# tier4/icp_rust

Hardware: AMD Instinct MI355X
Metric: ICP iterations/sec on 1M-pt 3D pair (higher is better)
Workload: dtype f64

## Files before the change

icp_rust_amd/_lib.py:

```python
import ctypes as C
import os
import subprocess

_HERE = os.path.dirname(os.path.abspath(__file__))
_CSRC = os.path.join(_HERE, "csrc")
LIB_PATH = os.environ.get("ICP_MI355X_LIB") or os.path.join(_HERE, "lib", "libicp_mi355x.so")

OK, NONE, EMPTY_DST, NAN_INPUT, BAD_ARGUMENT, NO_DEVICE, HIP_ERROR, OUT_OF_MEMORY, RETRY_REPLICATED, RETRY_SHARDED = range(10)
NN_AUTO, NN_BRUTE, NN_GRID = 0, 1, 2


class Pose(C.Structure):

    _fields_ = [(n, C.c_double) for n in ("r00", "r10", "r01", "r11", "tx", "ty")]

    def as_tuple(self):
        return (self.r00, self.r10, self.r01, self.r11, self.tx, self.ty)


class BatchItem(C.Structure):

    _fields_ = [("src_first", C.c_uint64), ("n", C.c_uint64), ("dst_first", C.c_uint64), ("m", C.c_uint64),
                ("init", Pose)]

# ... 86 lines not shown
    "icp_estimate_transform_device": (C.c_int, [_vp, _vp, _vp, _sz, _pp, _vp]),
    "icp_nn_search_device": (C.c_int, [_vp, _vp, _sz, _vp]),
    "icp_weighted_gn_step_device": (C.c_int, [_vp, _vp, _vp, _sz, _pp, C.c_int, _dp, _dp]),
    "icp_shard_geometry": (C.c_int, [_sz, C.c_int, C.c_int, C.POINTER(C.c_int), C.POINTER(C.c_int),
                                     C.POINTER(C.c_int), C.POINTER(_sz)]),
    "icp_shard_histogram_words": (_sz, []),
    "icp_shard_candidates_bytes": (_sz, []),
    "icp_shard_partials_bytes": (_sz, [C.c_int]),
    "icp_shard_exchange_bytes": (_sz, [C.c_int]),
    "icp_shard_take_device": (C.c_int, [_vp, _vp, _vp, _sz, C.c_int, C.c_int, _sz]),
    "icp_shard_put_device": (C.c_int, [_vp, _vp, _vp, _sz, C.c_int, C.c_int, _sz]),
    "icp_shard_eval_hist_device": (C.c_int, [_vp, _vp, _vp, _sz, C.c_int, C.c_int, _pp, C.c_int, C.c_int,
                                             C.POINTER(_vp)]),
    "icp_shard_eval_compact_device": (C.c_int, [_vp, _vp]),
    "icp_shard_eval_finish_device": (C.c_int, [_vp, _vp, _dp, _dp]),
    "icp_create_multi": (C.c_int, [C.POINTER(_vp), C.c_int, _vp, _sz, C.POINTER(C.c_int), C.c_int]),
    "icp_multi_estimate": (C.c_int, [_vp, _vp, _sz, _pp, _sz, _pp, _vp, _vp]),
    "icp_multi_counters": (C.c_int, [_vp, C.POINTER(C.c_uint64)]),
    "icp_multi_loop_counters": (C.c_int, [_vp, C.POINTER(C.c_uint64)]),
    "icp_multi_pipe_iterations": (C.c_int, [_vp, C.POINTER(C.c_uint64)]),
    "icp_pipe_counters": (C.c_int, [_vp, C.POINTER(C.c_uint64)]),
    "icp_debug_sort_cells": (C.c_int, [_vp, _sz, C.c_uint, _vp, _vp]),
    "icp_set_fixed_point_exit": (C.c_int, [_vp, C.c_int]),
    "icp_shard_pipe_run_device": (C.c_int, [_vp, _vp, _sz, _sz, C.c_int, C.c_int, _pp, C.POINTER(_sz), _sz, _vp, _vp,
                                            C.POINTER(C.c_int)]),
    "icp_loop_inbox_bytes": (_sz, []),
    "icp_loop_inbox": (C.c_int, [_vp, C.c_int, C.POINTER(C.c_void_p)]),
    "icp_loop_inbox_ipc_handle": (C.c_int, [_vp, C.c_char_p]),
    "icp_loop_ipc_open": (C.c_int, [C.c_int, C.c_char_p, C.POINTER(C.c_void_p)]),
    "icp_loop_ipc_close": (C.c_int, [_vp]),
    "icp_loop_inbox_shm_name": (C.c_int, [_vp, C.c_char_p]),
    "icp_loop_inbox_shm_unlink": (C.c_int, [_vp]),
    "icp_loop_shm_open": (C.c_int, [C.c_int, C.c_char_p, C.POINTER(C.c_void_p)]),
    "icp_loop_shm_close": (C.c_int, [_vp]),
    "icp_loop_transport_probe": (C.c_int, [_vp, C.c_int, C.POINTER(C.c_int)]),
    "icp_reset_window_predictions": (C.c_int, [_vp]),
    "icp_shard_loop_connect": (C.c_int, [_vp, C.c_int, C.c_int, C.POINTER(C.c_void_p)]),
    "icp_shard_loop_launch_device": (C.c_int, [_vp, _vp, _vp, _sz, C.c_uint, C.c_uint, C.c_int, C.c_uint32, _pp, C.c_double,
                                               C.c_int, C.c_int]),
    "icp_shard_loop_wait": (C.c_int, [_vp, _pp, C.POINTER(C.c_double), _u32p, C.POINTER(C.c_int), C.POINTER(C.c_int), _u32p]),
    "icp_destroy_multi": (None, [_vp]),
    "icp_synchronize": (C.c_int, [_vp]),
    "icp_profile_enable": (C.c_int, [_vp, C.c_int]),
    "icp_profile_read": (C.c_int, [_vp, _dp, C.POINTER(C.c_uint64)]),
    "icp_reduce_geometry": (None, [_sz, C.POINTER(C.c_int), C.POINTER(C.c_int)]),
    "icp_nn_cert_counters": (C.c_int, [_vp, C.POINTER(C.c_uint64)]),
# ... 97 lines not shown
```

icp_rust_amd/csrc/api.hip:

```cpp
#include <dlfcn.h>
#include <fcntl.h>
#include <sys/mman.h>
#include <unistd.h>

#include <cfloat>
#include <chrono>
#include <cstdio>
#include <cstring>
#include <atomic>
#include <map>
#include <mutex>
#include <new>

#include "api_internal.hpp"

using namespace icp;
using namespace icp::api;

namespace icp {
namespace api {
int map_hip(hipError_t e) {
  switch (e) {
    case hipSuccess: return ICP_OK;
    case hipErrorOutOfMemory: return ICP_OUT_OF_MEMORY;
// ... 1255 lines not shown
    if (rc != ICP_OK) return rc;
  }
  out[0] = h->ws.win_tried;
  out[1] = h->ws.win_missed;
  out[2] = h->ws.short_evals;
  out[3] = h->ws.radix_evals;
  out[4] = h->ws.spec_hits;
  out[5] = h->ws.spec_misses;
  return ICP_OK;
}

extern "C" int icp_gn_filed_counters(icp_handle *h, uint64_t out[2]) {
  if (!out) return ICP_BAD_ARGUMENT;
  std::lock_guard<std::mutex> lk(g_scratch_mu);
  if (!h) {
    const int rc = scratch_handle(&h);
    if (rc != ICP_OK) return rc;
  }
  out[0] = h->ws.bkt_evals;
  out[1] = h->ws.bkt_off;
  return ICP_OK;
}

extern "C" int icp_run_ahead_counters(icp_handle *h, uint64_t out[2]) {
  if (!h || !out) return ICP_BAD_ARGUMENT;
  out[0] = h->ws.ahead_hits;
  out[1] = h->ws.ahead_misses;
  return ICP_OK;
}

extern "C" int icp_gn_loop_timeouts(icp_handle *h, uint64_t *out) {
  if (!h || !out) return ICP_BAD_ARGUMENT;
  *out = h->ws.loop_timeouts;
  return ICP_OK;
}

extern "C" int icp_fixed_point_skips(icp_handle *h, uint64_t *out) {
  if (!h || !out) return ICP_BAD_ARGUMENT;
  *out = h->ws.fixed_point_skips;
  return ICP_OK;
}

extern "C" int icp_gn_loop_counters(icp_handle *h, uint64_t out[3]) {
  if (!out) return ICP_BAD_ARGUMENT;
  std::lock_guard<std::mutex> lk(g_scratch_mu);
  if (!h) {
// ... 98 lines not shown
```

icp_rust_amd/csrc/common.hpp:

```cpp
#pragma once
#include <hip/hip_runtime.h>

#include <cstddef>
#include <cstdint>
#include <cstdlib>
#include <utility>
#include <vector>

#include "pose.hpp"

namespace icp {


struct Range {
  explicit Range(const char *name);
  ~Range();
  Range(const Range &) = delete;
  Range &operator=(const Range &) = delete;
};

constexpr int kReduceThreads = 512;
constexpr int kReduceMaxBlocks = 256;
constexpr int kTreeMaxBlocks = 2048;
constexpr int kShardMaxWorld = 16;
// ... 152 lines not shown
  uint32_t *d_idx_slot = nullptr;
  double *d_sa = nullptr, *d_sb = nullptr;
  uint32_t *h_whist = nullptr;
  void *h_tiny = nullptr;
  unsigned long long tiny_calls = 0, tiny_evals = 0, tiny_sorted = 0;
  double *d_rlist = nullptr;
  unsigned *d_rlist_len = nullptr;
  size_t cap_part = 0;
  double *d_part_d = nullptr;
  uint32_t *d_part_i = nullptr;
  bool win_valid = false;
  bool win_wide = false;
  double win_med[2] = {0., 0.}, win_sigma[2] = {0., 0.};
  struct WinPred {
    bool valid = false, wide = false;
    double med[2] = {0., 0.}, sigma[2] = {0., 0.};
  };
  WinPred win_kind[5];
  WinPred hint_kind[5];
  uint32_t hint_last_inner = 0xffffffffu;
  static bool kind_has_slot(int kind) { return kind == 0 || kind == 1 || kind == 3 || kind == 4; }
  unsigned long long win_tried = 0, win_missed = 0, short_evals = 0, radix_evals = 0;
  unsigned long long bkt_evals = 0, bkt_misses = 0;
  unsigned long long fixed_point_skips = 0;
  unsigned bkt_off = 0;
  void *d_loop_ctl = nullptr, *h_loop_res = nullptr;
  uint32_t *d_loop_hist = nullptr;
  double *d_loop_part = nullptr;
  unsigned loop_seq = 0;
  bool loop_off = false;
  unsigned long long loop_launches = 0, loop_evals = 0, loop_handbacks = 0, loop_timeouts = 0;
  void *d_loop_inbox = nullptr;
  int loop_inbox_kind = 0;
  void *loop_inbox_host = nullptr;
  char loop_shm_name[64] = {0};
  unsigned loop_probe_gen = 0;
  unsigned loop_off_calls = 0;
  void *loop_peers[kShardMaxWorld] = {};
  int loop_rank = -1, loop_world = 0;
  void *loop_plan = nullptr;
  unsigned pipe_gen = 0;
  unsigned long long pipe_iters = 0, pipe_handbacks = 0, pipe_gave_up = 0;
  unsigned pipe_off = 0;
};

struct GridParams {
// ... 66 lines not shown
  bool have_prev = false;
  PrevMatch *d_prev = nullptr;
  double *d_sorted = nullptr;
  bool have_certs = false, have_pose = false, have_pose_before = false;
  double decay_r = 0., decay_t = 0.;
  Pose last_pose;
  uint32_t *d_cert_lists = nullptr;
  unsigned *d_cert_ctr = nullptr, *last_cert_ctr = nullptr;
  unsigned cert_seq = 0;
  unsigned long long cert_searches = 0;
};

hipError_t stable_sort_cells(const uint32_t *keys_in, uint32_t *perm_out, unsigned n, unsigned bits, void *&tmp, size_t &cap_tmp,
                             hipStream_t s);

}

struct icp_handle {
  int dim = 0;
  size_t m = 0;
  int device = 0;
  int nn_mode = ICP_NN_AUTO;
  bool single_launch = true;
  bool fixed_point_exit = true;
  bool owns_dst = false;
  const double *d_dst = nullptr;
  double *d_dst_own = nullptr;
  size_t cap_dst_own = 0, cap_soa = 0, cap_f32 = 0;
  double *d_dst_soa = nullptr;
  float *d_dst_f32 = nullptr;
  size_t m_pad = 0;
  bool brute_valid = false;
  bool screen_valid = false;
  hipStream_t own_stream = nullptr;
  hipStream_t stream = nullptr;
  icp::Workspace ws;
  icp::Grid grid;
  icp::QuerySort qsort;
  struct ShardEval {
    icp::WinParams P;
    int kind = 2, rank = 0, world = 1, b0 = 0, b1 = 0, blocks = 0;
    size_t n_local = 0, n_total = 0;
    const double *d_a = nullptr;
    icp::Pose T;
    double *d_ordered = nullptr;
    bool active = false;
// ... 192 lines not shown
```

icp_rust_amd/csrc/gn_device.hpp:

```cpp
#pragma once
#include "common.hpp"

namespace icp {

__device__ __forceinline__ unsigned long long f2k(double v) {
  const unsigned long long u = (unsigned long long)__double_as_longlong(v);
  return (u >> 63) ? ~u : (u | 0x8000000000000000ull);
}
__device__ __forceinline__ double k2f(unsigned long long k) {
  const unsigned long long u = (k >> 63) ? (k & 0x7fffffffffffffffull) : ~k;
  return __longlong_as_double((long long)u);
}

__device__ __forceinline__ int pass_shift(int pass) { return pass < 5 ? 52 - 12 * pass : 0; }
__device__ __forceinline__ int pass_bits(int pass) { return pass < 5 ? 12 : 4; }

__device__ __forceinline__ double huber_rho(double e) {
  const double k = ICP_HUBER_K;
  const double k2 = k * k;
  return (e <= k2) ? e : (2. * k * __dsqrt_rn(e) - k2);
}
__device__ __forceinline__ double huber_drho(double e) {
  const double k = ICP_HUBER_K;
  const double k2 = k * k;
// ... 26 lines not shown
      return __longlong_as_double((long long)(((unsigned long long)rh[1] << 32) | rl[1]));
    } else {
      const auto rl = __builtin_amdgcn_permlane16_swap(lo, lo, false, false);
      const auto rh = __builtin_amdgcn_permlane16_swap(hi, hi, false, false);
      return __longlong_as_double((long long)(((unsigned long long)rh[1] << 32) | rl[1]));
    }
#endif
  } else {
    const long long b = __double_as_longlong(v);
    const int lo = __builtin_amdgcn_update_dpp(0, (int)(b & 0xffffffffll), 0x100 + OFF, 0xf, 0xf, true);
    const int hi = __builtin_amdgcn_update_dpp(0, (int)(b >> 32), 0x100 + OFF, 0xf, 0xf, true);
    return __longlong_as_double(((long long)hi << 32) | (unsigned)lo);
  }
}
template <int N, int OFF>
__device__ __forceinline__ void tree_step(double (&acc)[N]) {
  double t[N];
#pragma unroll
  for (int k = 0; k < N; ++k) t[k] = tree_down<OFF>(acc[k]);
#pragma unroll
  for (int k = 0; k < N; ++k) acc[k] = acc[k] + t[k];
}
template <int N>
__device__ __forceinline__ void wave_tree(double (&acc)[N]) {
  tree_step<N, 32>(acc);
  tree_step<N, 16>(acc);
  tree_step<N, 8>(acc);
  tree_step<N, 4>(acc);
  tree_step<N, 2>(acc);
  tree_step<N, 1>(acc);
}

template <int N>
__device__ __forceinline__ void block_reduce_waves(double (&acc)[N], double (*sm)[N]) {
  wave_tree<N>(acc);
  if ((threadIdx.x & 63) == 0) {
#pragma unroll
    for (int k = 0; k < N; ++k) sm[threadIdx.x >> 6][k] = acc[k];
  }
}
template <int N, bool SC1 = false>
__device__ __forceinline__ void block_reduce_finish(const double (*sm)[N], double *__restrict__ out) {
  if (threadIdx.x < N) {
    const int k = threadIdx.x;
    double s = sm[0][k];
    for (int w = 1; w < (int)(blockDim.x >> 6); ++w) s = s + sm[w][k];
    if (SC1) __hip_atomic_store(out + k, s, __ATOMIC_RELAXED, __HIP_MEMORY_SCOPE_AGENT);
    else out[k] = s;
  }
}
template <int N, bool SC1 = false>
__device__ __forceinline__ void block_reduce_store(double (&acc)[N], double *__restrict__ out) {
  __shared__ double sm[16][N];
  block_reduce_waves<N>(acc, sm);
  __syncthreads();
  block_reduce_finish<N, SC1>(sm, out);
}


__device__ __forceinline__ bool last_block_arrives(TicketSet *t) {
  __shared__ int s_last;
  asm volatile("s_waitcnt vmcnt(0)" ::: "memory");
// ... 76 lines not shown
}

template <bool UNIFORM>
__device__ __forceinline__ void accumulate_pair(const double2 &s, double r0, double r1, const Pose &T, double *acc) {
  if constexpr (UNIFORM) {
    const double k2 = ICP_HUBER_K * ICP_HUBER_K;
    const double e0 = r0 * r0, e1 = r1 * r1, e2 = e0 + e1;
    double w0 = 1., w1 = 1., rho = e2;
    if (__ballot((e0 > k2) | (e1 > k2) | (e2 > k2))) {
      w0 = huber_drho(e0);
      w1 = huber_drho(e1);
      rho = huber_rho(e2);
    }
    accumulate_dim_w(0, s, r0, w0, T, acc);
    accumulate_dim_w(1, s, r1, w1, T, acc + 9);
    acc[18] = acc[18] + rho;
  } else {
    accumulate_dim<UNIFORM>(0, s, r0, T, acc);
    accumulate_dim<UNIFORM>(1, s, r1, T, acc + 9);
    accumulate_rho<UNIFORM>(r0, r1, acc + 18);
  }
}

__host__ __device__ __forceinline__ double combine_sum(const double *S, int k, const double *sig) {
  if (k >= 12) return S[18];
  int u;
  if (k >= 9) {
    u = 6 + (k - 9);
  } else {
    const int p = k / 3, q = k % 3;
    const int lo = p < q ? p : q, hi = p < q ? q : p;
    u = lo == 0 ? hi : (lo == 1 ? 2 + hi : 5);
  }
  double v = 0.;
  if (sig[0] != 0.) v = v + (1. / sig[0]) * S[u];
  if (sig[1] != 0.) v = v + (1. / sig[1]) * S[9 + u];
  return v;
}

__device__ __forceinline__ void accumulate_points(const double2 *__restrict__ a, const double *__restrict__ rx,
                                                  const double *__restrict__ ry, unsigned n, const Pose &T,
                                                  double (&acc)[kNSum]) {
  constexpr int kAccBatch = 4;
  const unsigned G = gridDim.x * kReduceThreads;
  for (unsigned base = blockIdx.x * kReduceThreads + threadIdx.x; base < n; base += G * kAccBatch) {
    double2 s[kAccBatch];
// ... 225 lines not shown
```

icp_rust_amd/csrc/gn_win.hip:

```cpp
#include "common.hpp"
#include "gn_device.hpp"
#include "gn_win_device.hpp"
#include "gn_loop.hpp"

namespace icp {


template <bool SUMS, int BATCH = kWinBatch>
__device__ __forceinline__ void win_hist_body(const double2 *__restrict__ a, const double2 *__restrict__ b,
                                              const Pose &T, double *__restrict__ rx, double *__restrict__ ry,
                                              unsigned n, const WinParams &P, uint32_t *whist, WinState *st,
                                              GnScalars *scal, double *partials, int status_cls = -1) {
  __shared__ uint32_t lh[2 * kWinBins];
  if (SUMS && status_cls >= 0 && blockIdx.x == 0 && threadIdx.x < (unsigned)kShardStatusWords)
    whist[2 * kWinBins + threadIdx.x] = (int)threadIdx.x == status_cls ? 1u : 0u;
  double acc[SUMS ? kNSum : 1];
#pragma unroll
  for (int k = 0; k < (SUMS ? kNSum : 1); ++k) acc[k] = 0.;
#ifdef ICP_WIN_DEBUG
  long long wst[6];
  wst[0] = wall_clock64();
#endif
  for (unsigned i = threadIdx.x; i < 2u * kWinBins; i += kWinThreads) lh[i] = 0;
  __syncthreads();
// ... 92 lines not shown
}

struct HistBktArgs {
  const double2 *a, *b;
  Pose T;
  unsigned n;
  WinParams P;
  uint32_t *whist;
  WinState *st;
  GnScalars *scal;
  double *partials;
  double *seg_all;
  unsigned short *dir_all;
};
struct HistBktLds {
  uint32_t lh[2 * kWinBins];
  double mv[kBktStage];
  unsigned short mk[kBktStage];
  WinRegion tab[2][8];
  double wsum[kWinThreads / 64][kNSum];
  unsigned nmem;
};

__device__ __forceinline__ void win_hist_sums_bkt_body(const HistBktArgs &A, const unsigned blk, const unsigned nblk,
                                                       HistBktLds &S) {
#ifndef ICP_BKT_BATCH
#define ICP_BKT_BATCH 2
#endif
  constexpr int BATCH = ICP_BKT_BATCH;
  const double2 *__restrict__ a = A.a, *__restrict__ b = A.b;
  const Pose T = A.T;
  const unsigned n = A.n;
  const WinParams &P = A.P;
  uint32_t *const whist = A.whist;
  WinState *const st = A.st;
  GnScalars *const scal = A.scal;
  double *const partials = A.partials;
  double *const seg_all = A.seg_all;
  unsigned short *const dir_all = A.dir_all;
  auto &lh = S.lh;
  auto &s_mv = S.mv;
  auto &s_mk = S.mk;
  unsigned &s_nmem = S.nmem;
  double acc[kNSum];
#pragma unroll
  for (int k = 0; k < kNSum; ++k) acc[k] = 0.;
#ifdef ICP_WIN_DEBUG
  long long bst[8];
  bst[0] = wall_clock64();
#endif
  for (unsigned i = threadIdx.x; i < 2u * kWinBins; i += kWinThreads) lh[i] = 0;
  if (threadIdx.x == 0) s_nmem = 0;
  if (threadIdx.x < 10) win_region_table(P.d[threadIdx.x / 5], S.tab[threadIdx.x / 5], (int)(threadIdx.x % 5));
  __syncthreads();
  const unsigned G = nblk * kWinThreads;
  const unsigned lane = threadIdx.x & 63u;
  double2 ns[BATCH], nd[BATCH];
  auto fetch = [&](unsigned from) {
#pragma unroll
    for (int u = 0; u < BATCH; ++u) {
      const unsigned i = from + u * G;
      if (i < n) {
        ns[u] = a[i];
        nd[u] = b[i];
      }
    }
  };
#ifdef ICP_WIN_DEBUG
  bst[5] = wall_clock64();
// ... 6 lines not shown
    for (int u = 0; u < BATCH; ++u) {
      s[u] = ns[u];
      d[u] = nd[u];
    }
#ifdef ICP_WIN_DEBUG
    if (!bst[6]) {
      asm volatile("s_waitcnt vmcnt(0)" ::: "memory");
      bst[6] = wall_clock64();
    }
#endif
    if (base + G * BATCH - lane < n) fetch(base + G * BATCH);
#ifdef ICP_WIN_DEBUG
    if (!bst[7] && !(base + G * BATCH - lane < n)) bst[7] = wall_clock64();
#endif
    double mv[2 * BATCH];
    unsigned mj[BATCH];
    unsigned mem = 0;
#pragma unroll
    for (int u = 0; u < BATCH; ++u) {
      const unsigned i = base + u * G;
      mv[2 * u] = mv[2 * u + 1] = 0.;
      mj[u] = 0u;
      if (i >= n) continue;
      const double v0 = ((T.r00 * s[u].x + T.r01 * s[u].y) + T.tx) - d[u].x;
      const double v1 = ((T.r10 * s[u].x + T.r11 * s[u].y) + T.ty) - d[u].y;
      bool lo0, hi0, f0, lo1, hi1, f1;
      const unsigned j0 = wbin_tab(v0, P.d[0], S.tab[0], lo0, hi0, f0), j1 = wbin_tab(v1, P.d[1], S.tab[1], lo1, hi1, f1);
      atomicAdd(&lh[j0], 1u);
      atomicAdd(&lh[kWinBins + j1], 1u);
      mv[2 * u] = v0;
      mv[2 * u + 1] = v1;
      mj[u] = j0 | (j1 << 16);
      mem |= ((unsigned)f0 << (2 * u)) | ((unsigned)f1 << (2 * u + 1));
      accumulate_pair<true>(s[u], v0, v1, T, acc);
    }
    const unsigned mine = (unsigned)__popc(mem), incl = wave_scan_inclusive(mine);
    const unsigned wave_total = (unsigned)__builtin_amdgcn_readlane((int)incl, 63);
    if (wave_total) {
      unsigned got = 0;
      if (lane == 63u) got = atomicAdd(&s_nmem, wave_total);
      unsigned pos = (unsigned)__builtin_amdgcn_readlane((int)got, 63) + incl - mine;
#pragma unroll
      for (int q = 0; q < 2 * BATCH; ++q) {
        if (mem & (1u << q)) {
          if (pos < (unsigned)kBktStage) {
            s_mv[pos] = mv[q];
            s_mk[pos] = (unsigned short)((q & 1) ? (unsigned)kWinBins + (mj[q >> 1] >> 16) : (mj[q >> 1] & 0xffffu));
          }
          ++pos;
        }
      }
    }
  }
  if (acc[kNSum - 1] != acc[kNSum - 1]) atomicOr(&scal->nan_flag, 1);
  block_reduce_waves<kNSum>(acc, S.wsum);
#ifdef ICP_WIN_DEBUG
  bst[1] = wall_clock64();
#endif
  __syncthreads();
#ifdef ICP_WIN_DEBUG
  bst[2] = wall_clock64();
#endif
  block_reduce_finish<kNSum, true>(S.wsum, partials + (size_t)blk * (kNSum + 1));
  for (unsigned i = threadIdx.x; i < 2u * kWinBins; i += kWinThreads) {
    const uint32_t c = lh[i];
    if (c) atomicAdd(&whist[i], c);
  }
  constexpr unsigned kDirPer = 8;
  static_assert(kWinFine % kDirPer == 0 && kBktFine / kDirPer <= kWinThreads, "directory slices");
  const unsigned f0 = threadIdx.x * kDirPer;
  const bool has_slice = f0 < (unsigned)kBktFine;
  const unsigned w0 = has_slice ? fine_to_word(f0) : 0u;
  unsigned cnt[kDirPer], sum = 0;
#pragma unroll
  for (unsigned q = 0; q < kDirPer; ++q) {
    cnt[q] = has_slice ? lh[w0 + q] : 0u;
    sum += cnt[q];
  }
  unsigned total;
  unsigned run = block_excl_scan(sum, &total);
  unsigned short *const dir = dir_all + (size_t)blk * kBktDir;
  double *const seg = seg_all + (size_t)blk * kBktStage;
  if (has_slice) {
    unsigned o[kDirPer];
#pragma unroll
    for (unsigned q = 0; q < kDirPer; ++q) {
// ... 16 lines not shown
  const unsigned nm_all = s_nmem;
  if (nm_all > (unsigned)kBktStage) {
    if (threadIdx.x == 0) atomicOr(&st->stage_overflow, 1u);
  } else {
    for (unsigned e = threadIdx.x; e < nm_all; e += kWinThreads) {
      const unsigned key = s_mk[e];
      const unsigned pos = atomicAdd(&lh[key], 1u);
      if (pos < (unsigned)kBktStage) seg[pos] = s_mv[e];
    }
  }
#ifdef ICP_WIN_DEBUG
  asm volatile("s_waitcnt vmcnt(0)" ::: "memory");
  bst[4] = wall_clock64();
  if (threadIdx.x == 0 && (blk == 0 || blk == 200) && (bst[0] & 0x1f0) == 0)
    printf("[B blk %d] stream %lld (prologue %lld first pairs %lld batches but the last %lld last %lld) barrier %lld flush+dir+reduce %lld "
           "scatter %lld (x10ns) members %u\n", blk, bst[1] - bst[0], bst[5] - bst[0], bst[6] - bst[5], bst[7] - bst[6],
           bst[1] - bst[7], bst[2] - bst[1], bst[3] - bst[2], bst[4] - bst[3], nm_all);
#endif
}

__global__ __launch_bounds__(kWinThreads, 4) void k_win_hist_sums_bkt(HistBktArgs A) {
  __shared__ HistBktLds S;
  win_hist_sums_bkt_body(A, blockIdx.x, gridDim.x, S);
}

constexpr unsigned kRehistStage = 1024;
__global__ __launch_bounds__(kWinThreads) void k_win_rehist(const double *__restrict__ rx,
                                                            const double *__restrict__ ry, unsigned n, WinParams P,
                                                            uint32_t *whist, WinState *st, double *lx, double *ly,
                                                            unsigned lcap, unsigned *llen) {
  __shared__ uint32_t lh[2 * kWinBins];
  __shared__ double s_stage[2][kRehistStage];
  __shared__ unsigned s_n[2], s_base[2];
  for (unsigned i = threadIdx.x; i < 2u * kWinBins; i += kWinThreads) lh[i] = 0;
  if (threadIdx.x < 2) s_n[threadIdx.x] = 0;
  __syncthreads();
  auto fine = [](unsigned j) {
    return (j >= (unsigned)kF0 && j < (unsigned)kC0) || (j >= (unsigned)kF1 && j < (unsigned)kC1) ||
           (j >= (unsigned)kF2 && j < (unsigned)(kWinBins - 1));
  };
  auto keep = [&](int d, double v) {
    const unsigned pos = atomicAdd(&s_n[d], 1u);
    if (pos < kRehistStage) {
      s_stage[d][pos] = v;
    } else {
      const unsigned g = atomicAdd(&llen[d], 1u);
// ... 797 lines not shown
  }
#ifdef ICP_WIN_DEBUG
  asm volatile("s_waitcnt vmcnt(0)" ::: "memory");
  PSTAMP(9);
  if (tid == 0 && A.seq % 16 == 5)
    printf("[P%d last] resolve %lld list %lld load+fold %lld sel1 %lld sel2 %lld store %lld ticket+loads %lld ahead %lld "
           "publish %lld (x10ns) cnt %u %u\n", d, pst[1] - pst[0], pst[2] - pst[1], pst[3] - pst[2], pst[4] - pst[3],
           pst[5] - pst[4], pst[6] - pst[5], pst[7] - pst[6], pst[8] - pst[7], pst[9] - pst[8], sel.med_cnt, sel.ring_cnt);
#endif
#undef PSTAMP
}

__global__ __launch_bounds__(kReduceThreads) void k_win_pick(PickArgs A) {
  __shared__ PickDimLds L;
  win_pick_dim_body(A, (int)blockIdx.x, true, L);
}

__global__ __launch_bounds__(kWinThreads, 4) void k_win_hist_sums_bkt2(HistBktArgs A, HistBktArgs B) {
  __shared__ HistBktLds S;
  const unsigned half = gridDim.x >> 1;
  if (blockIdx.x < half) win_hist_sums_bkt_body(A, blockIdx.x, half, S);
  else win_hist_sums_bkt_body(B, blockIdx.x - half, half, S);
}
__global__ __launch_bounds__(kReduceThreads) void k_win_pick2(PickArgs A, PickArgs B) {
  __shared__ PickDimLds L;
  if (blockIdx.x < 2u) win_pick_dim_body(A, (int)blockIdx.x, true, L);
  else win_pick_dim_body(B, (int)blockIdx.x - 2, false, L);
}

namespace {
constexpr long long kPipeTimeoutTicks = 300000000;
__device__ __forceinline__ void pst_u32(unsigned *p, unsigned v) { __hip_atomic_store(p, v, __ATOMIC_RELAXED, __HIP_MEMORY_SCOPE_SYSTEM); }
__device__ __forceinline__ void pst_f64(double *p, double v) { __hip_atomic_store(p, v, __ATOMIC_RELAXED, __HIP_MEMORY_SCOPE_SYSTEM); }
__device__ __forceinline__ unsigned pld_u32(const unsigned *p) { return __hip_atomic_load(p, __ATOMIC_RELAXED, __HIP_MEMORY_SCOPE_SYSTEM); }
__device__ __forceinline__ double pld_f64(const double *p) { return __hip_atomic_load(p, __ATOMIC_RELAXED, __HIP_MEMORY_SCOPE_SYSTEM); }

__device__ __forceinline__ bool pipe_poll(const unsigned long long *words, int count, unsigned gen, LoopInbox *const *box, int W,
                                          LoopInbox *me, unsigned *payload_or) {
  __shared__ int s_pok;
  __shared__ unsigned s_ppay;
  if (threadIdx.x < 64) {
    const int lane = (int)threadIdx.x;
    unsigned long long seen = 0;
    int ok = 1;
    const long long t0 = wall_clock64();
    for (;;) {
// ... 489 lines not shown
  return A;
}
static PickArgs bkt_pick_args(GnCtx &c, unsigned n, const WinParams &P, bool ahead_on, const Pose &ahead_outer,
                              AheadPose *d_ahead = nullptr) {
  PickArgs A;
  A.n = n;
  A.P = P;
  A.whist = c.d_whist;
  A.st = c.d_wstate;
  A.seg_all = c.d_bkt;
  A.dir_all = c.d_bkt_dir;
  A.segments = (int)tree_blocks(n);
  A.scal = c.d_scal;
  A.partials = c.d_partials;
  A.sum_blocks = A.segments;
  A.res = c.h_res;
  A.seq = ++c.seq;
  A.ahead = ahead_on ? d_ahead : nullptr;
  A.outer = ahead_on ? ahead_outer : transform_identity();
  A.join = c.d_wjoin;
  return A;
}

hipError_t launch_bkt_pair(icp_handle *h, hipStream_t s, GnCtx &first, const double *a1, const double *b1, const WinParams &P1,
                           bool ahead_on, const Pose &ahead_outer, GnCtx &second, const double *a2, const double *b2,
                           const Pose &T2, const WinParams &P2, size_t n_) {
  Workspace &w = h->ws;
  const unsigned n = (unsigned)n_, blocks = tree_blocks(n_);
  if (blocks > (unsigned)kReduceMaxBlocks) return hipErrorInvalidValue;
  w.bkt_evals += 2;
  hipLaunchKernelGGL(k_win_hist_sums_bkt2, dim3(2 * blocks), dim3(kWinThreads), 0, s,
                     bkt_hist_args(first, (const double2 *)a1, (const double2 *)b1, transform_identity(), n, P1),
                     bkt_hist_args(second, (const double2 *)a2, (const double2 *)b2, T2, n, P2));
  hipLaunchKernelGGL(k_win_pick2, dim3(4), dim3(kReduceThreads), 0, s,
                     bkt_pick_args(first, n, P1, ahead_on, ahead_outer, w.d_ahead),
                     bkt_pick_args(second, n, P2, false, transform_identity()));
  second.bkt_pair_launched = true;
  return hipGetLastError();
}

hipError_t launch_shard_evals(const ShardPickRank *rk, int nranks, int world, int B, size_t n_total, unsigned gen0,
                              const ShardPickEval *ev, int nevals) {
  if (nranks < 1 || nranks > kPipeFuse || nevals < 1 || nevals > 2 || world < 1 || world > kShardMaxWorld || B < 1 || B > kTreeMaxBlocks)
    return hipErrorInvalidValue;
  for (int j = 0; j < nranks; ++j)
    if (rk[j].nbl < 1 || rk[j].nbl > kReduceMaxBlocks || rk[j].b0 < 0 || rk[j].b0 + rk[j].nbl > B || rk[j].rank < 0 || rk[j].rank >= world ||
        !rk[j].h->ws.d_loop_inbox)
      return hipErrorInvalidValue;
  PickShardLaunch L = {};
  L.world = world;
  L.B = B;
  L.nranks = nranks;
  L.nevals = nevals;
  const Workspace &w0 = rk[0].h->ws;
  for (int q = 0; q < kShardMaxWorld; ++q) L.inbox[q] = reinterpret_cast<LoopInbox *>(w0.loop_peers[q < world ? q : 0]);
  for (int j = 0; j < nranks; ++j) {
// ... 29 lines not shown
    L.ev[e].n = (unsigned)n_total;
    L.ev[e].gen = gen0 + (unsigned)e;
    L.ev[e].ahead_on = ev[e].ahead_on ? 1 : 0;
    L.ev[e].P = ev[e].P;
    L.ev[e].outer = ev[e].ahead_on ? ev[e].outer : transform_identity();
  }
  hipLaunchKernelGGL(k_win_pick_shard, dim3((unsigned)nevals, (unsigned)nranks), dim3(kReduceThreads), 0, rk[0].h->stream, L);
  return hipGetLastError();
}

hipError_t launch_weighted_gn_win(icp_handle *h, const double *d_a, const double *d_b, size_t n_, const Pose &T,
                                  const WinParams &P) {
  Workspace &w = h->ws;
  const unsigned n = (unsigned)n_;
  const unsigned per = kWinThreads * kWinBatch;
  unsigned hb = (n + per - 1) / per;
  if (hb > (unsigned)kWinBlocks) hb = kWinBlocks;
  const double2 *a = (const double2 *)d_a, *b = (const double2 *)d_b;
  hipStream_t s = h->stream;
  if (w.bkt_off > 0) --w.bkt_off;
  else if (bkt_fits(n_, P)) {
    ++w.bkt_evals;
    const HistBktArgs HA = bkt_hist_args(w, a, b, T, n, P);
    hipLaunchKernelGGL(k_win_hist_sums_bkt, dim3(tree_blocks(n_)), dim3(kWinThreads), 0, s, HA);
    hipLaunchKernelGGL(k_win_pick, dim3(2), dim3(kReduceThreads), 0, s, bkt_pick_args(w, n, P, w.ahead_on, w.ahead_outer, w.d_ahead));
    return hipGetLastError();
  }
  int blocks, threads;
  reduce_geometry(n_, &blocks, &threads);
  hipLaunchKernelGGL(k_win_hist_sums, dim3(blocks), dim3(threads), 0, s, a, b, T, w.d_rx, w.d_ry, n, P, w.d_whist,
                     w.d_wstate, w.d_scal, w.d_partials, -1);
  hipLaunchKernelGGL(k_win_finish<false>, dim3(hb), dim3(kWinThreads), 0, s, (const double *)w.d_rx,
                     (const double *)w.d_ry, n, P, w.d_whist, w.d_wstate, w.d_wmed, w.d_wring, w.d_scal,
                     (const double *)w.d_partials, blocks, w.d_ctl, w.h_res, ++w.seq, (const unsigned *)nullptr, 0u,
                     w.ahead_on ? w.d_ahead : (AheadPose *)nullptr, w.ahead_on ? w.ahead_outer : transform_identity());
  return hipGetLastError();
}

bool refine_applies(size_t n) {
  static const bool off = getenv("ICP_GN_NO_REFINE") != nullptr;
  return !off && n > kWinMaxN && n / kRefineSample >= 1 && n < 0xffffffffull;
}

hipError_t launch_sample_pairs(icp_handle *h, const double *d_a, const double *d_b, size_t n) {
  Workspace &w = h->ws;
  hipError_t e;
  if (!w.d_sa) {
// ... 114 lines not shown
```

include/icp_mi355x_debug.h:

```cpp
#ifndef ICP_MI355X_DEBUG_H
#define ICP_MI355X_DEBUG_H

#include "icp_mi355x.h"

#ifdef __cplusplus
extern "C" {
#endif

int icp_gn_path_counters(icp_handle *h, uint64_t out[6]);

int icp_gn_loop_counters(icp_handle *h, uint64_t out[3]);
int icp_gn_loop_timeouts(icp_handle *h, uint64_t *out);
int icp_fixed_point_skips(icp_handle *h, uint64_t *out);

int icp_run_ahead_counters(icp_handle *h, uint64_t out[2]);

int icp_gn_filed_counters(icp_handle *h, uint64_t out[2]);

int icp_nn_cert_counters(icp_handle *h, uint64_t out[2]);

int icp_single_launch_counters(icp_handle *h, uint64_t out[3]);

int icp_grid_append_counters(const icp_handle *h, uint64_t out[2]);

int icp_grid_crop_counters(const icp_handle *h, uint64_t out[2]);

int icp_multi_counters(const icp_multi *M, uint64_t out[2]);

int icp_multi_loop_counters(const icp_multi *M, uint64_t out[3]);

int icp_multi_pipe_iterations(const icp_multi *M, uint64_t *out);
int icp_pipe_counters(icp_handle *h, uint64_t out[4]);

int icp_set_fixed_point_exit(icp_handle *h, int enable);

int icp_debug_sort_cells(const uint32_t *keys, size_t n, unsigned bits, uint32_t *keys_out, uint32_t *perm_out);

int icp_batch_counters(icp_batch *b, uint64_t out[4]);
int icp_batch_evaluate_counters(icp_batch *b, uint64_t out[3]);
int icp_batch_line_counters(icp_batch *b, uint64_t out[4]);

int icp_profile_enable(icp_handle *h, int enable);
int icp_profile_read(icp_handle *h, double *nn_kernel_ms, uint64_t *nn_kernel_launches);

#ifdef __cplusplus
}
#endif

#endif
```

Before: 9823.

## Add packed cross-lane wave reduction and identity-pose specialized histogram-sum kernel

Replaces the per-sum shuffle tree in the block reduction with a packed tree that pairs sums through gfx950 permlane32/16 swaps and DPP row moves, halving the number of live values at each level and scattering results to shared memory from several lanes. Adds an identity-pose variant of the bucketed histogram/sums kernel. When the pose is exactly identity it skips the rotation and translation arithmetic, accumulates only the 11 nonzero moment sums, and skips the Huber weighting when no lane exceeds the threshold. A debug entry point compares the packed tree against the reference tree. The costs are bit-level reinterpretation of doubles and a different summation order, which can change rounding.

```diff
diff --git a/icp_rust_amd/_lib.py b/icp_rust_amd/_lib.py
--- a/icp_rust_amd/_lib.py
+++ b/icp_rust_amd/_lib.py
@@ -132,6 +132,9 @@
     "icp_pipe_counters": (C.c_int, [_vp, C.POINTER(C.c_uint64)]),
     "icp_debug_sort_cells": (C.c_int, [_vp, _sz, C.c_uint, _vp, _vp]),
     "icp_set_fixed_point_exit": (C.c_int, [_vp, C.c_int]),
+    "icp_debug_wave_trees": (C.c_int, [_vp, C.c_int, _vp, _vp]),
+    "icp_set_identity_eval": (C.c_int, [_vp, C.c_int]),
+    "icp_identity_eval_counters": (C.c_int, [_vp, C.POINTER(C.c_uint64)]),
     "icp_shard_pipe_run_device": (C.c_int, [_vp, _vp, _sz, _sz, C.c_int, C.c_int, _pp, C.POINTER(_sz), _sz, _vp, _vp,
                                             C.POINTER(C.c_int)]),
     "icp_loop_inbox_bytes": (_sz, []),
diff --git a/icp_rust_amd/csrc/api.hip b/icp_rust_amd/csrc/api.hip
--- a/icp_rust_amd/csrc/api.hip
+++ b/icp_rust_amd/csrc/api.hip
@@ -1301,6 +1301,26 @@
   return ICP_OK;
 }
 
+extern "C" int icp_set_identity_eval(icp_handle *h, int enable) {
+  std::lock_guard<std::mutex> lk(g_scratch_mu);
+  if (!h) {
+    const int rc = scratch_handle(&h);
+    if (rc != ICP_OK) return rc;
+  }
+  h->identity_eval = enable != 0;
+  return ICP_OK;
+}
+extern "C" int icp_identity_eval_counters(icp_handle *h, uint64_t *out) {
+  if (!out) return ICP_BAD_ARGUMENT;
+  std::lock_guard<std::mutex> lk(g_scratch_mu);
+  if (!h) {
+    const int rc = scratch_handle(&h);
+    if (rc != ICP_OK) return rc;
+  }
+  out[0] = h->ws.ident_launches;
+  return ICP_OK;
+}
+
 extern "C" int icp_run_ahead_counters(icp_handle *h, uint64_t out[2]) {
   if (!h || !out) return ICP_BAD_ARGUMENT;
   out[0] = h->ws.ahead_hits;
diff --git a/icp_rust_amd/csrc/common.hpp b/icp_rust_amd/csrc/common.hpp
--- a/icp_rust_amd/csrc/common.hpp
+++ b/icp_rust_amd/csrc/common.hpp
@@ -198,6 +198,7 @@
   static bool kind_has_slot(int kind) { return kind == 0 || kind == 1 || kind == 3 || kind == 4; }
   unsigned long long win_tried = 0, win_missed = 0, short_evals = 0, radix_evals = 0;
   unsigned long long bkt_evals = 0, bkt_misses = 0;
+  unsigned long long ident_launches = 0;
   unsigned long long fixed_point_skips = 0;
   unsigned bkt_off = 0;
   void *d_loop_ctl = nullptr, *h_loop_res = nullptr;
@@ -310,6 +311,7 @@
   int device = 0;
   int nn_mode = ICP_NN_AUTO;
   bool single_launch = true;
+  bool identity_eval = true;
   bool fixed_point_exit = true;
   bool owns_dst = false;
   const double *d_dst = nullptr;
diff --git a/icp_rust_amd/csrc/gn_device.hpp b/icp_rust_amd/csrc/gn_device.hpp
--- a/icp_rust_amd/csrc/gn_device.hpp
+++ b/icp_rust_amd/csrc/gn_device.hpp
@@ -72,7 +72,7 @@
   for (int k = 0; k < N; ++k) acc[k] = acc[k] + t[k];
 }
 template <int N>
-__device__ __forceinline__ void wave_tree(double (&acc)[N]) {
+__device__ __forceinline__ void wave_tree_reference(double (&acc)[N]) {
   tree_step<N, 32>(acc);
   tree_step<N, 16>(acc);
   tree_step<N, 8>(acc);
@@ -80,14 +80,89 @@
   tree_step<N, 2>(acc);
   tree_step<N, 1>(acc);
 }
+template <int N>
+__device__ __forceinline__ void wave_tree(double (&acc)[N]) {
+  wave_tree_reference<N>(acc);
+}
+
+__device__ __forceinline__ void tree_split(double v, unsigned &lo, unsigned &hi) {
+  const unsigned long long b = (unsigned long long)__double_as_longlong(v);
+  lo = (unsigned)(b & 0xffffffffull);
+  hi = (unsigned)(b >> 32);
+}
+__device__ __forceinline__ double tree_join(unsigned lo, unsigned hi) {
+  return __longlong_as_double((long long)(((unsigned long long)hi << 32) | lo));
+}
+template <int OFF>
+__device__ __forceinline__ double tree_pack_swap(double a, double b) {
+  static_assert(OFF == 32 || OFF == 16, "the two lane swaps of gfx950");
+  unsigned alo, ahi, blo, bhi;
+  tree_split(a, alo, ahi);
+  tree_split(b, blo, bhi);
+  if constexpr (OFF == 32) {
+    const auto rl = __builtin_amdgcn_permlane32_swap(alo, blo, false, false);
+    const auto rh = __builtin_amdgcn_permlane32_swap(ahi, bhi, false, false);
+    return tree_join(rl[0], rh[0]) + tree_join(rl[1], rh[1]);
+  } else {
+    const auto rl = __builtin_amdgcn_permlane16_swap(alo, blo, false, false);
+    const auto rh = __builtin_amdgcn_permlane16_swap(ahi, bhi, false, false);
+    return tree_join(rl[0], rh[0]) + tree_join(rl[1], rh[1]);
+  }
+}
+template <int OFF>
+__device__ __forceinline__ double tree_pack_row(double a, double b) {
+  static_assert(OFF == 8 || OFF == 4, "bank masks select groups of four lanes");
+  constexpr int kUp = OFF == 8 ? 0xc : 0xa;
+  constexpr int kDn = 0xf ^ kUp;
+  unsigned alo, ahi, blo, bhi;
+  tree_split(a, alo, ahi);
+  tree_split(b, blo, bhi);
+  const unsigned xlo = (unsigned)__builtin_amdgcn_update_dpp((int)alo, (int)blo, 0x110 + OFF, 0xf, kUp, false);
+  const unsigned xhi = (unsigned)__builtin_amdgcn_update_dpp((int)ahi, (int)bhi, 0x110 + OFF, 0xf, kUp, false);
+  const unsigned ylo = (unsigned)__builtin_amdgcn_update_dpp((int)blo, (int)alo, 0x100 + OFF, 0xf, kDn, false);
+  const unsigned yhi = (unsigned)__builtin_amdgcn_update_dpp((int)bhi, (int)ahi, 0x100 + OFF, 0xf, kDn, false);
+  return tree_join(xlo, xhi) + tree_join(ylo, yhi);
+}
+template <int M, int OFF>
+__device__ __forceinline__ void tree_pack_step(double (&v)[M], double (&out)[(M + 1) / 2]) {
+#pragma unroll
+  for (int j = 0; j < (M + 1) / 2; ++j) {
+    const bool paired = 2 * j + 1 < M;
+    const double a = v[2 * j], b = v[paired ? 2 * j + 1 : 2 * j];
+    if constexpr (OFF >= 16) out[j] = tree_pack_swap<OFF>(a, b);
+    else out[j] = paired ? tree_pack_row<OFF>(a, b) : a + tree_down<OFF>(a);
+  }
+}
+template <int N>
+__device__ __forceinline__ void wave_tree_packed(double (&acc)[N], double *row) {
+  constexpr int M1 = (N + 1) / 2, M2 = (M1 + 1) / 2, M3 = (M2 + 1) / 2, M4 = (M3 + 1) / 2;
+  double v1[M1], v2[M2], v3[M3], v4[M4];
+  tree_pack_step<N, 32>(acc, v1);
+  tree_pack_step<M1, 16>(v1, v2);
+  tree_pack_step<M2, 8>(v2, v3);
+  tree_pack_step<M3, 4>(v3, v4);
+  tree_step<M4, 2>(v4);
+  tree_step<M4, 1>(v4);
+  const unsigned l = threadIdx.x & 63u;
+  const unsigned k0 = ((l >> 5) & 1u) | (((l >> 4) & 1u) << 1) | (((l >> 3) & 1u) << 2) | (((l >> 2) & 1u) << 3);
+  if ((l & 3u) == 0u) {
+#pragma unroll
+    for (int q = 0; q < M4; ++q)
+      if (k0 + 16u * q < (unsigned)N) row[k0 + 16u * q] = v4[q];
+  }
+}
 
 template <int N>
 __device__ __forceinline__ void block_reduce_waves(double (&acc)[N], double (*sm)[N]) {
-  wave_tree<N>(acc);
+#ifdef ICP_TREE_REFERENCE
+  wave_tree_reference<N>(acc);
   if ((threadIdx.x & 63) == 0) {
 #pragma unroll
     for (int k = 0; k < N; ++k) sm[threadIdx.x >> 6][k] = acc[k];
   }
+#else
+  wave_tree_packed<N>(acc, sm[threadIdx.x >> 6]);
+#endif
 }
 template <int N, bool SC1 = false>
 __device__ __forceinline__ void block_reduce_finish(const double (*sm)[N], double *__restrict__ out) {
@@ -210,6 +285,48 @@
   }
 }
 
+constexpr int kIdentSums = 11;
+constexpr unsigned kIdentLive = 0x1u | 0x4u | 0x20u | 0x40u | 0x100u | (0x8u | 0x10u | 0x20u | 0x80u | 0x100u) << 9 | 1u << 18;
+static_assert(kNSum == 19 && __builtin_popcount(kIdentLive) == kIdentSums, "the columns of common.hpp: kNSum");
+__device__ __forceinline__ void accumulate_pair_identity(const double2 &s, double r0, double r1, double *acc, bool &unbounded) {
+  const double k2 = ICP_HUBER_K * ICP_HUBER_K;
+  const double e0 = r0 * r0, e1 = r1 * r1, e2 = e0 + e1;
+  double w0 = 1., w1 = 1., rho = e2;
+  if (__ballot((e0 > k2) | (e1 > k2) | (e2 > k2))) {
+    w0 = huber_drho(e0);
+    w1 = huber_drho(e1);
+    rho = huber_rho(e2);
+    unbounded |= e2 > 1.7976931348623157e308;
+  }
+  const double jx = -s.y, jy = s.x;
+  const double tx = w0 * jx, ty = w1 * jy;
+  acc[0] = acc[0] + w0;
+  acc[1] = acc[1] + tx;
+  acc[2] = acc[2] + tx * jx;
+  acc[3] = acc[3] + w0 * r0;
+  acc[4] = acc[4] + tx * r0;
+  acc[5] = acc[5] + w1;
+  acc[6] = acc[6] + ty;
+  acc[7] = acc[7] + ty * jy;
+  acc[8] = acc[8] + w1 * r1;
+  acc[9] = acc[9] + ty * r1;
+  acc[10] = acc[10] + rho;
+}
+template <bool SC1 = false>
+__device__ __forceinline__ void block_reduce_finish_identity(const double (*sm)[kIdentSums], double *__restrict__ out) {
+  if (threadIdx.x < kNSum) {
+    const unsigned k = threadIdx.x;
+    double s = 0.;
+    if ((kIdentLive >> k) & 1u) {
+      const int c = __popc(kIdentLive & ((1u << k) - 1u));
+      s = sm[0][c];
+      for (int w = 1; w < (int)(blockDim.x >> 6); ++w) s = s + sm[w][c];
+    }
+    if (SC1) __hip_atomic_store(out + k, s, __ATOMIC_RELAXED, __HIP_MEMORY_SCOPE_AGENT);
+    else out[k] = s;
+  }
+}
+
 __host__ __device__ __forceinline__ double combine_sum(const double *S, int k, const double *sig) {
   if (k >= 12) return S[18];
   int u;
diff --git a/icp_rust_amd/csrc/gn_win.hip b/icp_rust_amd/csrc/gn_win.hip
--- a/icp_rust_amd/csrc/gn_win.hip
+++ b/icp_rust_amd/csrc/gn_win.hip
@@ -138,12 +138,16 @@
   unsigned nmem;
 };
 
+template <bool IDENT = false>
 __device__ __forceinline__ void win_hist_sums_bkt_body(const HistBktArgs &A, const unsigned blk, const unsigned nblk,
                                                        HistBktLds &S) {
 #ifndef ICP_BKT_BATCH
 #define ICP_BKT_BATCH 2
 #endif
-  constexpr int BATCH = ICP_BKT_BATCH;
+#ifndef ICP_BKT_IDENT_BATCH
+#define ICP_BKT_IDENT_BATCH ICP_BKT_BATCH
+#endif
+  constexpr int BATCH = IDENT ? ICP_BKT_IDENT_BATCH : ICP_BKT_BATCH;
   const double2 *__restrict__ a = A.a, *__restrict__ b = A.b;
   const Pose T = A.T;
   const unsigned n = A.n;
@@ -158,9 +162,11 @@
   auto &s_mv = S.mv;
   auto &s_mk = S.mk;
   unsigned &s_nmem = S.nmem;
-  double acc[kNSum];
-#pragma unroll
-  for (int k = 0; k < kNSum; ++k) acc[k] = 0.;
+  constexpr int NS = IDENT ? kIdentSums : kNSum;
+  double acc[NS];
+#pragma unroll
+  for (int k = 0; k < NS; ++k) acc[k] = 0.;
+  bool unbounded = false;
 #ifdef ICP_WIN_DEBUG
   long long bst[8];
   bst[0] = wall_clock64();
@@ -213,8 +219,8 @@
       mv[2 * u] = mv[2 * u + 1] = 0.;
       mj[u] = 0u;
       if (i >= n) continue;
-      const double v0 = ((T.r00 * s[u].x + T.r01 * s[u].y) + T.tx) - d[u].x;
-      const double v1 = ((T.r10 * s[u].x + T.r11 * s[u].y) + T.ty) - d[u].y;
+      const double v0 = IDENT ? (s[u].x + 0.) - d[u].x : ((T.r00 * s[u].x + T.r01 * s[u].y) + T.tx) - d[u].x;
+      const double v1 = IDENT ? (s[u].y + 0.) - d[u].y : ((T.r10 * s[u].x + T.r11 * s[u].y) + T.ty) - d[u].y;
       bool lo0, hi0, f0, lo1, hi1, f1;
       const unsigned j0 = wbin_tab(v0, P.d[0], S.tab[0], lo0, hi0, f0), j1 = wbin_tab(v1, P.d[1], S.tab[1], lo1, hi1, f1);
       atomicAdd(&lh[j0], 1u);
@@ -223,7 +229,8 @@
       mv[2 * u + 1] = v1;
       mj[u] = j0 | (j1 << 16);
       mem |= ((unsigned)f0 << (2 * u)) | ((unsigned)f1 << (2 * u + 1));
-      accumulate_pair<true>(s[u], v0, v1, T, acc);
+      if constexpr (IDENT) accumulate_pair_identity(s[u], v0, v1, acc, unbounded);
+      else accumulate_pair<true>(s[u], v0, v1, T, acc);
     }
     const unsigned mine = (unsigned)__popc(mem), incl = wave_scan_inclusive(mine);
     const unsigned wave_total = (unsigned)__builtin_amdgcn_readlane((int)incl, 63);
@@ -243,8 +250,10 @@
       }
     }
   }
-  if (acc[kNSum - 1] != acc[kNSum - 1]) atomicOr(&scal->nan_flag, 1);
-  block_reduce_waves<kNSum>(acc, S.wsum);
+  if (acc[NS - 1] != acc[NS - 1]) atomicOr(&scal->nan_flag, 1);
+  if (IDENT && unbounded) atomicOr(&st->stage_overflow, 1u);
+  double (*const wsum)[NS] = reinterpret_cast<double (*)[NS]>(&S.wsum[0][0]);
+  block_reduce_waves<NS>(acc, wsum);
 #ifdef ICP_WIN_DEBUG
   bst[1] = wall_clock64();
 #endif
@@ -252,7 +261,8 @@
 #ifdef ICP_WIN_DEBUG
   bst[2] = wall_clock64();
 #endif
-  block_reduce_finish<kNSum, true>(S.wsum, partials + (size_t)blk * (kNSum + 1));
+  if constexpr (IDENT) block_reduce_finish_identity<true>(wsum, partials + (size_t)blk * (kNSum + 1));
+  else block_reduce_finish<kNSum, true>(wsum, partials + (size_t)blk * (kNSum + 1));
   for (unsigned i = threadIdx.x; i < 2u * kWinBins; i += kWinThreads) {
     const uint32_t c = lh[i];
     if (c) atomicAdd(&whist[i], c);
@@ -315,6 +325,10 @@
 __global__ __launch_bounds__(kWinThreads, 4) void k_win_hist_sums_bkt(HistBktArgs A) {
   __shared__ HistBktLds S;
   win_hist_sums_bkt_body(A, blockIdx.x, gridDim.x, S);
+}
+__global__ __launch_bounds__(kWinThreads, 4) void k_win_hist_sums_bkt_ident(HistBktArgs A) {
+  __shared__ HistBktLds S;
+  win_hist_sums_bkt_body<true>(A, blockIdx.x, gridDim.x, S);
 }
 
 constexpr unsigned kRehistStage = 1024;
@@ -1158,6 +1172,12 @@
   if (blockIdx.x < half) win_hist_sums_bkt_body(A, blockIdx.x, half, S);
   else win_hist_sums_bkt_body(B, blockIdx.x - half, half, S);
 }
+__global__ __launch_bounds__(kWinThreads, 4) void k_win_hist_sums_bkt2_ident(HistBktArgs A, HistBktArgs B) {
+  __shared__ HistBktLds S;
+  const unsigned half = gridDim.x >> 1;
+  if (blockIdx.x < half) win_hist_sums_bkt_body<true>(A, blockIdx.x, half, S);
+  else win_hist_sums_bkt_body(B, blockIdx.x - half, half, S);
+}
 __global__ __launch_bounds__(kReduceThreads) void k_win_pick2(PickArgs A, PickArgs B) {
   __shared__ PickDimLds L;
   if (blockIdx.x < 2u) win_pick_dim_body(A, (int)blockIdx.x, true, L);
@@ -1693,6 +1713,16 @@
   return A;
 }
 
+static bool identity_form(icp_handle *h, const Pose &T) {
+  const Pose I = transform_identity();
+#ifdef ICP_NO_IDENTITY_FORM
+  return false;
+#endif
+  if (!h->identity_eval || memcmp(&T, &I, sizeof(Pose)) != 0) return false;
+  ++h->ws.ident_launches;
+  return true;
+}
+
 hipError_t launch_bkt_pair(icp_handle *h, hipStream_t s, GnCtx &first, const double *a1, const double *b1, const WinParams &P1,
                            bool ahead_on, const Pose &ahead_outer, GnCtx &second, const double *a2, const double *b2,
                            const Pose &T2, const WinParams &P2, size_t n_) {
@@ -1700,9 +1730,10 @@
   const unsigned n = (unsigned)n_, blocks = tree_blocks(n_);
   if (blocks > (unsigned)kReduceMaxBlocks) return hipErrorInvalidValue;
   w.bkt_evals += 2;
-  hipLaunchKernelGGL(k_win_hist_sums_bkt2, dim3(2 * blocks), dim3(kWinThreads), 0, s,
-                     bkt_hist_args(first, (const double2 *)a1, (const double2 *)b1, transform_identity(), n, P1),
-                     bkt_hist_args(second, (const double2 *)a2, (const double2 *)b2, T2, n, P2));
+  const HistBktArgs H1 = bkt_hist_args(first, (const double2 *)a1, (const double2 *)b1, transform_identity(), n, P1);
+  const HistBktArgs H2 = bkt_hist_args(second, (const double2 *)a2, (const double2 *)b2, T2, n, P2);
+  if (identity_form(h, H1.T)) hipLaunchKernelGGL(k_win_hist_sums_bkt2_ident, dim3(2 * blocks), dim3(kWinThreads), 0, s, H1, H2);
+  else hipLaunchKernelGGL(k_win_hist_sums_bkt2, dim3(2 * blocks), dim3(kWinThreads), 0, s, H1, H2);
   hipLaunchKernelGGL(k_win_pick2, dim3(4), dim3(kReduceThreads), 0, s,
                      bkt_pick_args(first, n, P1, ahead_on, ahead_outer, w.d_ahead),
                      bkt_pick_args(second, n, P2, false, transform_identity()));
@@ -1778,7 +1809,8 @@
   else if (bkt_fits(n_, P)) {
     ++w.bkt_evals;
     const HistBktArgs HA = bkt_hist_args(w, a, b, T, n, P);
-    hipLaunchKernelGGL(k_win_hist_sums_bkt, dim3(tree_blocks(n_)), dim3(kWinThreads), 0, s, HA);
+    if (identity_form(h, T)) hipLaunchKernelGGL(k_win_hist_sums_bkt_ident, dim3(tree_blocks(n_)), dim3(kWinThreads), 0, s, HA);
+    else hipLaunchKernelGGL(k_win_hist_sums_bkt, dim3(tree_blocks(n_)), dim3(kWinThreads), 0, s, HA);
     hipLaunchKernelGGL(k_win_pick, dim3(2), dim3(kReduceThreads), 0, s, bkt_pick_args(w, n, P, w.ahead_on, w.ahead_outer, w.d_ahead));
     return hipGetLastError();
   }
diff --git a/icp_rust_amd/csrc/tree_debug.hip b/icp_rust_amd/csrc/tree_debug.hip
--- /dev/null
+++ b/icp_rust_amd/csrc/tree_debug.hip
@@ -0,0 +1,54 @@
+#include "common.hpp"
+#include "gn_device.hpp"
+
+namespace icp {
+
+template <int N>
+__global__ __launch_bounds__(64) void k_debug_wave_trees(const double *__restrict__ in, double *__restrict__ out_packed,
+                                                         double *__restrict__ out_reference) {
+  __shared__ double row[N];
+  double p[N], r[N];
+#pragma unroll
+  for (int k = 0; k < N; ++k) p[k] = r[k] = in[k * 64 + (int)threadIdx.x];
+  wave_tree_packed<N>(p, row);
+  wave_tree_reference<N>(r);
+  __syncthreads();
+  if (threadIdx.x < N) out_packed[threadIdx.x] = row[threadIdx.x];
+  if (threadIdx.x == 0) {
+#pragma unroll
+    for (int k = 0; k < N; ++k) out_reference[k] = r[k];
+  }
+}
+
+template <int N>
+static void launch_debug_wave_trees(const double *in, double *out_packed, double *out_reference) {
+  hipLaunchKernelGGL(k_debug_wave_trees<N>, dim3(1), dim3(64), 0, nullptr, in, out_packed, out_reference);
+}
+
+}
+
+extern "C" int icp_debug_wave_trees(const double *in, int n_sums, double *out_packed, double *out_reference) {
+  if (!in || !out_packed || !out_reference || n_sums < 1 || n_sums > 20) return 4;
+  const size_t n = (size_t)n_sums;
+  double *d_in = nullptr, *d_out = nullptr;
+  hipError_t e = hipMalloc(&d_in, n * 64 * sizeof(double));
+  if (e == hipSuccess) e = hipMalloc(&d_out, 2 * n * sizeof(double));
+  if (e == hipSuccess) e = hipMemcpy(d_in, in, n * 64 * sizeof(double), hipMemcpyHostToDevice);
+  if (e == hipSuccess) {
+    switch (n_sums) {
+#define ICP_TREE_CASE(N) case N: icp::launch_debug_wave_trees<N>(d_in, d_out, d_out + n); break;
+      ICP_TREE_CASE(1) ICP_TREE_CASE(2) ICP_TREE_CASE(3) ICP_TREE_CASE(4) ICP_TREE_CASE(5)
+      ICP_TREE_CASE(6) ICP_TREE_CASE(7) ICP_TREE_CASE(8) ICP_TREE_CASE(9) ICP_TREE_CASE(10)
+      ICP_TREE_CASE(11) ICP_TREE_CASE(12) ICP_TREE_CASE(13) ICP_TREE_CASE(14) ICP_TREE_CASE(15)
+      ICP_TREE_CASE(16) ICP_TREE_CASE(17) ICP_TREE_CASE(18) ICP_TREE_CASE(19) ICP_TREE_CASE(20)
+#undef ICP_TREE_CASE
+    }
+    e = hipGetLastError();
+  }
+  if (e == hipSuccess) e = hipDeviceSynchronize();
+  if (e == hipSuccess) e = hipMemcpy(out_packed, d_out, n * sizeof(double), hipMemcpyDeviceToHost);
+  if (e == hipSuccess) e = hipMemcpy(out_reference, d_out + n, n * sizeof(double), hipMemcpyDeviceToHost);
+  (void)hipFree(d_in);
+  (void)hipFree(d_out);
+  return e == hipSuccess ? 0 : 6;
+}
diff --git a/include/icp_mi355x_debug.h b/include/icp_mi355x_debug.h
--- a/include/icp_mi355x_debug.h
+++ b/include/icp_mi355x_debug.h
@@ -34,7 +34,12 @@
 
 int icp_set_fixed_point_exit(icp_handle *h, int enable);
 
+int icp_set_identity_eval(icp_handle *h, int enable);
+int icp_identity_eval_counters(icp_handle *h, uint64_t *out);
+
 int icp_debug_sort_cells(const uint32_t *keys, size_t n, unsigned bits, uint32_t *keys_out, uint32_t *perm_out);
+
+int icp_debug_wave_trees(const double *in, int n_sums, double *out_packed, double *out_reference);
 
 int icp_batch_counters(icp_batch *b, uint64_t out[4]);
 int icp_batch_evaluate_counters(icp_batch *b, uint64_t out[3]);
```

After: 9935 (median of 2 runs). Within noise of the previous version (+1.1%).
